# ZackAttack614/BlackBird

Hardware: AMD Instinct MI355X
Metric: selfplay_games_per_sec (higher is better)
Workload: dtype f32 (float32 operands split exactly into 3 bf16 values, 6 bf16 MFMA products each, f32 accumulate)

## Files before the change

### blackbird_amd/csrc/mega2.hip.h

```cpp
#pragma once
#include "net.hip.h"
#include "net_x3.hip.h"
#include "tree.hip.h"

#define MEGA_RMAX 4
#define MEGA_HEAD_FLOATS 192

#define MEGA2_QCAP 32
#ifndef BB_TREE_IDLE_SLEEP
#define BB_TREE_IDLE_SLEEP 4
#endif
#ifndef BB_NET_IDLE_SLEEP
#define BB_NET_IDLE_SLEEP 4
#endif

__device__ __forceinline__ int lds_load(volatile int *p) { return *p; }
__device__ __forceinline__ void release_global_then_lds() {
    __threadfence_block();
    asm volatile("s_waitcnt vmcnt(0)" ::: "memory");
}


template <class G, int GW, bool REC>
struct GameShadow {
    static constexpr int S = G::S, MP = G::MAXPATH;
    int32_t root[GW], root_N[GW], n_nodes[GW], ply[GW], sims_left[GW], pend_leaf[GW], pend_expand[GW], path_len[GW],
        game_lid[GW], sim_serial[GW], leaf_serial[GW], resume_cur[GW], resume_depth[GW], leaf_flags[GW];
    int32_t path_N[REC ? GW * MP : 1], path_all[REC ? GW * MP : 1];
    float path_W[REC ? GW * MP : 1];
    uint32_t leaf_game_id[GW];
    float root_W[GW], eval_value[GW];
    float eval_policy[GW * S];
    uint64_t evals[GW];
    uint64_t ctr[GW * 8];
    typename G::State leaf_state[GW];
    uint32_t path[GW * MP];
    int8_t root_pp[GW];

#define BB_SHADOW_ARRAYS(X)                                                                                           \
    X(root, 1) X(root_N, 1) X(n_nodes, 1) X(ply, 1) X(sims_left, 1) X(pend_leaf, 1) X(pend_expand, 1) X(path_len, 1)  \
    X(game_lid, 1) X(sim_serial, 1) X(leaf_serial, 1) X(resume_cur, 1) X(resume_depth, 1) X(leaf_game_id, 1)          \
    X(root_W, 1) X(eval_value, 1) X(eval_policy, S) X(evals, 1) X(ctr, 8) X(path, MP) X(root_pp, 1) X(leaf_flags, 1)
#define BB_SHADOW_REC_ARRAYS(X) X(path_N, MP) X(path_all, MP) X(path_W, MP)

    __device__ __forceinline__ void load(const TreeDev &d, int g0, int n, int nthreads) {
#define X(f, per) for (int i = threadIdx.x; i < n * (per); i += nthreads) f[i] = d.f[(size_t)g0 * (per) + i];
        BB_SHADOW_ARRAYS(X)
        if constexpr (REC) { BB_SHADOW_REC_ARRAYS(X) }
#undef X
        for (int i = threadIdx.x; i < n; i += nthreads) leaf_state[i] = ((const typename G::State *)d.leaf_state)[g0 + i];
    }
    __device__ __forceinline__ void store(const TreeDev &d, int g0, int n, int nthreads) {
#define X(f, per) for (int i = threadIdx.x; i < n * (per); i += nthreads) d.f[(size_t)g0 * (per) + i] = f[i];
        BB_SHADOW_ARRAYS(X)
        if constexpr (REC) { BB_SHADOW_REC_ARRAYS(X) }
#undef X
        for (int i = threadIdx.x; i < n; i += nthreads) ((typename G::State *)d.leaf_state)[g0 + i] = leaf_state[i];
    }
    __device__ __forceinline__ TreeDev local(const TreeDev &d, int g0) {
        TreeDev r = d;
#define X(f, per) r.f = f;
        BB_SHADOW_ARRAYS(X)
        if constexpr (REC) { BB_SHADOW_REC_ARRAYS(X) }
#undef X
        r.leaf_state = leaf_state;
        r.pool_g0 = g0;
        return r;
    }
};

struct QueueCtl {
    int q[MEGA2_QCAP];
    int head, tail, tree_done, abort_flag;
};

__device__ __attribute__((noinline)) int queue_pop(QueueCtl *c, long long t_start, long long t_limit, int n_tree) {
    int li = -1;
    if ((threadIdx.x & 63) == 0) {
        int h = lds_load(&c->head), t = lds_load(&c->tail);
        if (h < t) {
            if (atomicCAS(&c->head, h, h + 1) == h) {
                volatile int *slot = &c->q[h & (MEGA2_QCAP - 1)];
                for (int spin = 0; spin < (1 << 20) && (li = *slot) < 0; spin++) __builtin_amdgcn_s_sleep(1);
                *slot = -1;
                if (li < 0) {
                    c->abort_flag = 1;
                    li = -2;
                }
            }
        } else if (lds_load(&c->tree_done) >= n_tree) {
            li = -2;
        } else if (wall_clock64() - t_start > t_limit || lds_load(&c->abort_flag)) {
            c->abort_flag = 1;
            li = -2;
        }
    }
    return __builtin_amdgcn_readfirstlane(li);
}

template <bool GLOBAL_TOO>
__device__ __attribute__((noinline)) void queue_push(QueueCtl *c, uint8_t *state_byte, bool leader, bool posted, int li) {
    if (GLOBAL_TOO) release_global_then_lds();
    else __threadfence_block();
    if (leader) {
        if (posted) {
            *(volatile uint8_t *)state_byte = 1;
            int idx = atomicAdd(&c->tail, 1);
            *(volatile int *)&c->q[idx & (MEGA2_QCAP - 1)] = li;
        } else {
            *(volatile uint8_t *)state_byte = 0;
        }
    }
}

template <class G, int NETW, bool X3 = false, int WAVES = 12>
__global__ void __launch_bounds__(WAVES * 64) k_selfplay_queue(TreeDev dg, NetDev nd, NetX3 x3, int noise_on, int limit_s, int own_visits) {
    constexpr int MEGA2_THREADS = WAVES * 64;
    constexpr bool NET_APPLIES = !X3;
    constexpr int S = G::S, GW = 16, TREEW = WAVES - NETW, GPT = (GW + TREEW - 1) / TREEW;
    static_assert(GPT * S <= 64, "a tree wave holds at most 64 / S games");
    using NG = NetGeom<G, 1>;
    constexpr int RMAX = MEGA_RMAX, STEPS0 = NG::STEPS0;
    using XG = X3Geom<G>;
    constexpr int EPI_F = (1 + 2 * RMAX) * 48, HEAD_F = MEGA_HEAD_FLOATS;
    constexpr int WT_F = X3 ? 2 * RMAX * XG::LAYER12_B / 4 : 2 * RMAX * 9 * 64 * 4, W0_F = X3 ? XG::W0_B / 4 : STEPS0 * 64;
    constexpr int WAVE_F = X3 ? XG::WAVE_BYTES / 4 : NG::WAVE_FLOATS;
    __shared__ __attribute__((aligned(16))) float lds[NETW * WAVE_F];
    constexpr int WH_F = X3 ? 3 * 64 * 16 / 4 : 0;
    __shared__ __attribute__((aligned(16))) float wlds[WT_F + W0_F + EPI_F + HEAD_F + WH_F];
    __shared__ QueueCtl qc;
    __shared__ GameShadow<G, GW, X3> shadow;
    static_assert(GPT <= 8, "a tree wave's game states are one 8-byte word");
    __shared__ __attribute__((aligned(8))) uint8_t gstate[TREEW * 8];
#define GSI(li) ((((li) % TREEW) << 3) + (li) / TREEW)
    __shared__ int myslot[NETW];
    __shared__ int wg_pool, wg_dry, wg_refill;
    constexpr int CHUNK = GW * 32;
#ifdef BB_STAMPS
    __shared__ long long ts_post[GW], ts_done[GW];
#endif
    const int wave = threadIdx.x >> 6, l64 = threadIdx.x & 63;
    const int g0 = blockIdx.x * GW;
    const int n_mine = dg.n_slots - g0 < GW ? dg.n_slots - g0 : GW;
    shadow.load(dg, g0, n_mine, MEGA2_THREADS);
    const TreeDev d = shadow.local(dg, g0);
    if (threadIdx.x == 0) {
        qc.head = 0;
        qc.tail = 0;
        qc.tree_done = 0;
        qc.abort_flag = 0;
        wg_pool = n_mine * own_visits;
        wg_dry = 0;
        wg_refill = 0;
    }
    if (threadIdx.x < TREEW * 8) gstate[threadIdx.x] = 0;
#ifdef BB_STAMPS_NET
    if (threadIdx.x < 8) s_net_stamps[threadIdx.x] = 0;
#endif
    if (threadIdx.x < MEGA2_QCAP) qc.q[threadIdx.x] = -1;
    for (int i = threadIdx.x; i < NETW * WAVE_F; i += MEGA2_THREADS) lds[i] = 0.f;
    NetDev ndl = nd;
    NetX3 x3l = x3;
    {
        const float *gwt = X3 ? (const float *)x3.wt12 : (const float *)nd.wt;
        const float *gw0 = X3 ? (const float *)x3.w0 : nd.w0;
        const int wt_used = X3 ? 2 * nd.R * XG::LAYER12_B / 4 : 2 * nd.R * 9 * 64 * 4;
        for (int i = threadIdx.x; i < wt_used; i += MEGA2_THREADS) wlds[i] = gwt[i];
        for (int i = threadIdx.x; i < W0_F; i += MEGA2_THREADS) wlds[WT_F + i] = gw0[i];
        x3l.wt12 = (const unsigned char *)wlds;
        x3l.w0 = (const unsigned char *)(wlds + WT_F);
        for (int i = threadIdx.x; i < (1 + 2 * nd.R) * 48; i += MEGA2_THREADS) wlds[WT_F + W0_F + i] = nd.epi[i];
        for (int i = threadIdx.x; i < nd.head_floats; i += MEGA2_THREADS) wlds[WT_F + W0_F + EPI_F + i] = nd.head[i];
        if constexpr (X3) {
            for (int i = threadIdx.x; i < WH_F; i += MEGA2_THREADS) wlds[WT_F + W0_F + EPI_F + HEAD_F + i] = ((const float *)x3.wh)[i];
            x3l.wh = (const unsigned char *)(wlds + WT_F + W0_F + EPI_F + HEAD_F);
        }
        ndl.wt = (const f32x4 *)wlds;
        ndl.w0 = wlds + WT_F;
        ndl.epi = wlds + WT_F + W0_F;
        ndl.head = wlds + WT_F + W0_F + EPI_F;
    }
    __syncthreads();
    const long long t_start = wall_clock64();
    const long long t_limit = 100000000ll * limit_s;

    if (wave >= NETW) {
        const int tw = wave - NETW;
        __builtin_amdgcn_s_setprio(3);
        const int li = (l64 / S) * TREEW + tw, lane = l64 % S;
        const bool mine = l64 < GPT * S && li < GW && g0 + li < d.n_slots;
        const int g = li;
        bool alive = mine && d.game_lid[mine ? g : 0] >= 0;
#ifdef BB_STAMPS
        long long t_work = 0, t_all0 = clock64(), n_calls = 0, n_lanes = 0, t_pick = 0, n_pick = 0;
#endif
        auto early_post = [&](int gg, int ln) __attribute__((always_inline)) {
            if (NET_APPLIES) release_global_then_lds();
            else __threadfence_block();
            if (ln == 0) {
#ifdef BB_STAMPS
                ts_post[li] = wall_clock64();
#endif
                *(volatile uint8_t *)&gstate[GSI(li)] = 1;
                const int idx = atomicAdd(&qc.tail, 1);
                *(volatile int *)&qc.q[idx & (MEGA2_QCAP - 1)] = li;
            }
        };
        for (;;) {
            int stt = mine ? (int)*(volatile uint8_t *)&gstate[GSI(li)] : 1;
            const int pool = lds_load(&wg_pool), dry = lds_load(&wg_dry);
            if (pool < CHUNK / 4 && !dry && __any(alive)) {
                if (l64 == 0 && atomicCAS(&wg_refill, 0, 1) == 0) {
                    int old = atomicSub(d.visit_pool, CHUNK);
                    int got = old < 0 ? 0 : old < CHUNK ? old : CHUNK;
                    if (got) atomicAdd(&wg_pool, got);
                    else *(volatile int *)&wg_dry = 1;
                    __threadfence_block();
                    *(volatile int *)&wg_refill = 0;
                }
                if (pool <= 0) {
                    __builtin_amdgcn_s_sleep(1);
                    int late = wall_clock64() - t_start > t_limit || lds_load(&qc.abort_flag);
                    if (__builtin_amdgcn_readfirstlane(late)) {
                        qc.abort_flag = 1;
                        break;
                    }
                    continue;
                }
            }
            bool ready = mine && alive && pool > 0 && stt != 1;
            bool busy = mine && ((alive && pool > 0) || (alive && !dry) || stt == 1);
            if (!__any(busy)) break;
            if (__any(ready)) {
                __threadfence_block();
                bool posted = false;
#ifdef BB_STAMPS
                long long ts = clock64();
                n_calls++;
                n_lanes += __popcll(__ballot(ready)) / S;
                if (ready && lane == 0 && stt == 2) {
                    t_pick += wall_clock64() - ts_done[li];
                    n_pick++;
                }
#endif
#ifdef BB_STAMPS_LIGHT
                int ll = 0, lv = 0, lld = 0, lpu = 0;
                if (ready) {
                    posted = async_game<G, X3>(d, g, lane, ll, lv, lld, lpu, early_post);
                    if (d.game_lid[g] < 0) alive = false;
                }
                {
                    int m = lv;
                    for (int o = 32; o; o >>= 1) m = max(m, __shfl_xor(m, o, 64));
                    unsigned long long who = __ballot(ready && lane == 0 && lv == m);
                    if (who && l64 == (int)__builtin_ctzll(who) && d.stamps) {
                        atomicAdd(&d.stamps[6], (unsigned long long)ll);
                        atomicAdd(&d.stamps[7], (unsigned long long)lv);
                        atomicAdd(&d.stamps[11], (unsigned long long)lld);
                        atomicAdd(&d.stamps[12], (unsigned long long)lpu);
                    }
                }
#else
                if (ready) {
                    posted = async_game<G, X3>(d, g, lane, early_post);
                    if (d.game_lid[g] < 0) alive = false;
                }
#endif
                {
                    int used = __popcll(__ballot(ready && lane == 0));
                    if (l64 == 0) atomicSub(&wg_pool, used);
                }
                queue_push<NET_APPLIES>(&qc, &gstate[GSI(li < GW ? li : 0)], ready && lane == 0 && !posted, false, li);
#ifdef BB_STAMPS
                t_work += clock64() - ts;
#endif
            } else {
                __builtin_amdgcn_s_sleep(BB_TREE_IDLE_SLEEP);
                int late = wall_clock64() - t_start > t_limit || lds_load(&qc.abort_flag);
                if (__builtin_amdgcn_readfirstlane(late)) {
                    qc.abort_flag = 1;
                    break;
                }
            }
        }
        if (l64 == 0) atomicAdd(&qc.tree_done, 1);
#ifdef BB_STAMPS
        if (l64 == 0 && d.stamps) {
            atomicAdd(&d.stamps[2], (unsigned long long)t_work);
            atomicAdd(&d.stamps[3], (unsigned long long)(clock64() - t_all0));
            atomicAdd(&d.stamps[5], 1ull);
            atomicAdd(&d.stamps[13], (unsigned long long)n_calls);
            atomicAdd(&d.stamps[14], (unsigned long long)n_lanes);
        }
        if (lane == 0 && d.stamps && n_pick) {
            atomicAdd(&d.stamps[8], (unsigned long long)t_pick);
            atomicAdd(&d.stamps[9], (unsigned long long)n_pick);
        }
#endif
    } else {
        float *wl = lds + wave * WAVE_F;
        constexpr bool CACHE = X3 && G::CACHE_KEY;
        const EvalCache ecache = {(u32x4 *)dg.eval_cache, dg.eval_cache_log2};
        unsigned long long n_probes = 0, n_hits = 0;
#ifdef BB_STAMPS
        long long t_work = 0, t_all0 = clock64(), n_evals = 0, t_qwait = 0;
#endif
        for (;;) {
            const int li = __builtin_amdgcn_readfirstlane(queue_pop(&qc, t_start, t_limit, TREEW));
            if (li == -2) break;
            if (li < 0) {
                __builtin_amdgcn_s_sleep(BB_NET_IDLE_SLEEP);
                continue;
            }
            __threadfence_block();
#ifdef BB_STAMPS
            long long ts = clock64();
            n_evals++;
            t_qwait += wall_clock64() - ts_post[li];
#endif
            if (l64 == 0) myslot[wave] = li;
            if constexpr (X3) {
                int probe = -1;
                net_body_x3<G, true, false, CACHE>(ndl, x3l, 1, 0, &myslot[wave], (unsigned char *)wl, (const typename G::State *)d.leaf_state, nullptr,
                                     d.leaf_game_id, d.leaf_serial, noise_on, d.eval_value, nullptr, d.eval_policy, S, false, nullptr,
                                     ecache, &probe);
                if constexpr (CACHE) {
                    n_probes += probe >= 0;
                    if (probe > 0) {
                        n_hits++;
                        if (l64 == 0) d.evals[li] -= 1;
                    }
                }
            } else
                net_body<G, 1, 2>(ndl, 1, 0, &myslot[wave], wl, (const typename G::State *)d.leaf_state, nullptr,
                                  d.leaf_game_id, d.leaf_serial, noise_on, d.eval_value, nullptr, d.eval_policy, S, false);
            if constexpr (NET_APPLIES) {
            __threadfence_block();
#ifdef BB_STAMPS_NET
            long long _na = clock64();
#endif
            if (l64 < S) {
                phase_apply<G>(d, li, l64);
                if (l64 == 0) d.sims_left[li] -= 1;
            }
#ifdef BB_STAMPS_NET
            if (l64 == 0) atomicAdd(&s_net_stamps[5], (unsigned long long)(clock64() - _na));
#endif
            }
            release_global_then_lds();
#ifdef BB_STAMPS
            if (l64 == 0) ts_done[li] = wall_clock64();
#endif
            if (l64 == 0) *(volatile uint8_t *)&gstate[GSI(li)] = 2;
#ifdef BB_STAMPS
            t_work += clock64() - ts;
#endif
        }
#ifdef BB_STAMPS
        if (l64 == 0 && d.stamps) {
            atomicAdd(&d.stamps[0], (unsigned long long)t_work);
            atomicAdd(&d.stamps[1], (unsigned long long)(clock64() - t_all0));
            atomicAdd(&d.stamps[4], 1ull);
            atomicAdd(&d.stamps[15], (unsigned long long)n_evals);
            atomicAdd(&d.stamps[10], (unsigned long long)t_qwait);
        }
#endif
        if (CACHE && l64 == 0 && n_probes && dg.eval_cache_ctr) {
            atomicAdd(&dg.eval_cache_ctr[0], n_hits);
            atomicAdd(&dg.eval_cache_ctr[1], n_probes);
        }
    }
    __syncthreads();
#ifdef BB_STAMPS_NET
    if (threadIdx.x < 8) atomicAdd(&g_net_stamps[threadIdx.x], s_net_stamps[threadIdx.x]);
#endif
    if (qc.abort_flag) {
        if (threadIdx.x == 0) d.ctr[6] += 1;
        if ((int)threadIdx.x < n_mine && gstate[GSI(threadIdx.x)] == 1) shadow.pend_leaf[threadIdx.x] = -1;
    }
    __syncthreads();
    shadow.store(dg, g0, n_mine, MEGA2_THREADS);
}
```

### blackbird_amd/csrc/tree.hip.h

```cpp
#pragma once
#include "games.hip.h"
#include "rng.hip.h"

#define NODE_EXPANDED 1
#define NODE_TERMINAL 2
#define NODE_CACHED 4
#define LEAF_RECORDED 0x40000000
#define CHILD_NONE (-1)
#define CHILD_TERM_BIT 0x40000000

template <class G>
struct alignas(128) DenseNode {
    int32_t flags;
    uint32_t legal_mask;
    int32_t all;
    int32_t serial;
    double sq;
    double pad0;
    int32_t N[G::S];
    float Q[G::S];
    int32_t child[G::S];
    alignas(128) double cP[G::S];
    float W[G::S];
    typename G::State st;
// ... 696 lines not shown
    pool->serial = 0;
    d.n_nodes[g] = 1;
    d.root[g] = 0;
    d.root_N[g] = 0;
    d.root_W[g] = 0.f;
    d.root_pp[g] = 0;
    d.ply[g] = 0;
    d.pend_leaf[g] = -1;
    d.pend_expand[g] = 0;
    d.path_len[g] = 0;
    d.sim_serial[g] = 0;
    d.game_lid[g] = lid;
    if (d.leaf_flags) d.leaf_flags[g] = 0;
    if (d.track_anc) {
        d.anc_len[g] = 0;
        d.top_N[g] = 0;
    }
}

template <class G>
__global__ void __launch_bounds__(256) k_set_roots(TreeDev d, int n, const int32_t *slots,
                                                   const typename G::State *states, const uint32_t *game_ids) {
    int i = blockIdx.x * blockDim.x + threadIdx.x;
    if (i >= n) return;
    int g = slots ? slots[i] : i;
    if (g < 0 || g >= d.n_slots) return;
    reset_slot<G>(d, g, game_ids ? (int)game_ids[i] : g, states[i]);
    d.sims_left[g] = 0;
}

template <class G>
__global__ void __launch_bounds__(256) k_add_sims(TreeDev d, int sims, const uint8_t *mask = nullptr) {
    int g = blockIdx.x * blockDim.x + threadIdx.x;
    if (g >= d.n_slots) return;
    if (d.game_lid[g] >= 0 && (!mask || mask[g])) d.sims_left[g] = sims;
}

template <class G>
__global__ void __launch_bounds__(256) k_get_roots(TreeDev d, typename G::State *out) {
    int g = blockIdx.x * blockDim.x + threadIdx.x;
    if (g >= d.n_slots) return;
    out[g] = ((DenseNode<G> *)d.nodes + (size_t)(g + d.pool_g0) * d.node_cap + d.root[g])->st;
}

template <class G>
__global__ void __launch_bounds__(256) k_selfplay_begin(TreeDev d) {
    int g = blockIdx.x * blockDim.x + threadIdx.x;
    if (g >= d.n_slots) return;
    if (g + d.slot_offset < d.n_games_target) {
        reset_slot<G>(d, g, g + d.slot_offset, G::initial());
        d.sims_left[g] = d.sims_per_move;
    } else {
        reset_slot<G>(d, g, -1, G::initial());
        d.sims_left[g] = 0;
    }
}

template <class G>
__device__ __forceinline__ uint8_t *example_ptr(const TreeDev &d, int lid, int ply) {
    return d.examples + ((size_t)lid * (d.max_plies + 1) + ply) * d.example_bytes;
}

template <class G>
__device__ __forceinline__ void write_example(const TreeDev &d, int lid, int ply, const typename G::State &st, int lane, int Ni,
                              int total, uint32_t gid) {
    uint8_t *p = example_ptr<G>(d, lid, ply);
    if (lane == 0) {
        ExampleHdr h;
        h.game_id = gid;
        h.ply = (uint16_t)ply;
        h.player = (uint8_t)gs_player(st);
        h.z = 0;
        h.total = (uint32_t)total;
        h.n_children = G::A;
        *(ExampleHdr *)p = h;
        *(typename G::State *)(p + sizeof(ExampleHdr)) = st;
    }
    ((uint32_t *)(p + sizeof(ExampleHdr) + sizeof(typename G::State)))[lane] = (uint32_t)Ni;
}

template <class G>
__device__ __forceinline__ void selfplay_move_body(const TreeDev &d, int g, int lane) {
    using Node = DenseNode<G>;
    constexpr int S = G::S;
    int lid = d.game_lid[g];
    if (lid < 0) return;
    Node *pool = (Node *)d.nodes + (size_t)(g + d.pool_g0) * d.node_cap;
    typename G::State st = pool[d.root[g]].st;
    uint32_t gid = d.first_game_id + (uint32_t)lid;
    int ply = d.ply[g];
    double u = bb_u53(d.seed, gid, (uint32_t)ply);
    int total, Ni;
    float Wi;
    int act = choose_move<G>(d, g, lane, d.temp, u, total, Ni, Wi);
    if (act < 0) {
        if (lane == 0) {
            d.game_lid[g] = -1;
            d.ctr[(size_t)g * 8 + 6] += 1;
        }
        return;
    }
    write_example<G>(d, lid, ply, st, lane, Ni, total, gid);
    typename G::State ns;
    advance_root<G>(d, g, lane, act, ns);
    __threadfence_block();
    ply += 1;
    int w = G::winner(ns, -1);
    bool over = w >= 0 || ply >= d.max_plies;
    if (!over) {
        if (lane == 0) {
            d.ply[g] = ply;
            d.sims_left[g] = d.sims_per_move;
            d.ctr[(size_t)g * 8 + 5] += 1;
        }
        return;
    }
    write_example<G>(d, lid, ply, ns, lane, 0, 0, gid);
    __threadfence_block();
    for (int k = lane; k <= ply; k += S) {
        ExampleHdr *h = (ExampleHdr *)example_ptr<G>(d, lid, k);
        h->z = (w <= 0) ? 0 : (h->player == w ? 1 : -1);
    }
    __threadfence();
    if (lane == 0) {
        int32_t *gh = d.game_hdr + (size_t)lid * 4;
        gh[0] = ply + 1;
        gh[1] = w;
        gh[2] = ply;
        __threadfence();
        gh[3] = 1;
        uint64_t *c = d.ctr + (size_t)g * 8;
        c[4] += 1;
        c[5] += 1;
        c[7] += (uint64_t)(ply + 1);
        int next = lid + d.lid_stride;
        if (next < d.n_games_target) {
            reset_slot<G>(d, g, next, G::initial());
            d.sims_left[g] = d.sims_per_move;
        } else {
            d.game_lid[g] = -1;
            d.sims_left[g] = 0;
        }
    }
}

template <class G>
__global__ void __launch_bounds__(256) k_selfplay_move(TreeDev d) {
    constexpr int S = G::S;
    int t = blockIdx.x * blockDim.x + threadIdx.x;
    int g = t / S, lane = t % S;
    if (g >= d.n_slots) return;
    phase_apply<G>(d, g, lane);
    __threadfence_block();
    selfplay_move_body<G>(d, g, lane);
}

struct NoPostHook {
    __device__ __forceinline__ void operator()(int, int) const {}
};
template <class G, bool REC = false, class OnPost = NoPostHook>
__device__ bool async_game(const TreeDev &d, int g, int lane
#ifdef BB_STAMPS_LIGHT
                           , int &g_light_loop, int &g_light_levels, int &g_light_load, int &g_light_puct
#endif
                           , OnPost on_post = OnPost()) {
    using Node = DenseNode<G>;
    constexpr int S = G::S, A = G::A;
    if (d.game_lid[g] < 0) return false;
    Node *pool = (Node *)d.nodes + (size_t)(g + d.pool_g0) * d.node_cap;
#ifdef BB_STAMPS_LIGHT
    int lt_in = (int)clock64(), lt_loop = 0, ln_levels = 0, lt_create = 0, lt_puct = 0;
#endif
    if (d.pend_leaf[g] >= 0) {
        if (REC && (d.leaf_flags[g] & LEAF_RECORDED)) phase_apply_rec<G>(d, g, lane);
        else phase_apply<G>(d, g, lane);
        if (lane == 0) d.sims_left[g] -= 1;
        __threadfence_block();
    }
    int budget = d.level_budget;
    uint32_t *path = d.path + (size_t)g * G::MAXPATH;
    int sims_done = 0, depth_sum = 0, term_hits = 0;
    bool posted = false;
    for (;;) {
        if (d.sims_left[g] <= 0) {
            selfplay_move_body<G>(d, g, lane);
            __threadfence_block();
            if (d.game_lid[g] < 0) break;
        }
        int cur = d.resume_cur[g], depth = 0;
        if (cur >= 0) depth = d.resume_depth[g];
        else cur = d.root[g];
        int nn = d.n_nodes[g];
        typename G::State st;
        int flags = 0;
        enum { F_PARKED = 2, F_LEAF = 4, F_TERM = 8, F_EXPAND = 16, F_OVERFLOW = 32 };
        int fl = 0;
#ifdef BB_STAMPS_LIGHT
        int lt_e = (int)clock64();
#endif
        for (;;) {
            if (budget <= 0) { fl |= F_PARKED; break; }
            budget--;
#ifdef BB_STAMPS_LIGHT
            ln_levels++;
            int lt_a = (int)clock64();
#endif
            Node *node = pool + cur;
            typename G::State st_l = node->st;
            int flags_l = node->flags;
            uint32_t mask = node->legal_mask;
            double sq = node->sq;
            int Ni = node->N[lane];
            float Qi = node->Q[lane];
            double cPi = node->cP[lane];
            int ci = node->child[lane];
            double cached = node->pad0;
            float Wi = 0.f;
            int all_l = 0;
            if (REC) {
                Wi = node->W[lane];
                all_l = node->all;
            }
            asm volatile("" ::"v"(flags_l), "v"(mask), "v"(sq), "v"(Ni), "v"(Qi), "v"(cPi), "v"(ci));
#ifdef BB_STAMPS_LIGHT
            int lt_b = (int)clock64();
            lt_create += lt_b - lt_a;
#endif
            st = st_l;
            flags = flags_l;
            if (!(flags & NODE_EXPANDED)) {
                fl |= F_LEAF;
                if (flags & NODE_TERMINAL) {
                    fl |= F_TERM;
                    if (flags & NODE_CACHED) {
                        float v01 = (float)cached;
                        __threadfence_block();
                        if (REC) backup_path_rec<G>(d, g, lane, pool, depth, v01, gs_prev(st));
                        else backup_path<G>(d, g, lane, pool, depth, v01, gs_prev(st));
                        if (lane == 0) d.sims_left[g] -= 1;
                        __threadfence_block();
                        sims_done++;
                        depth_sum += depth;
                        term_hits++;
                        fl &= ~F_LEAF;
                    }
                } else {
                    fl |= F_EXPAND;
                }
                break;
            }
            static_assert(G::MAXPATH >= G::H * G::W + 2, "a descent places at most H*W stones");
            int child = ci;
            int a = grp_argmax_puct<S>(Qi, cPi, sq, Ni, lane < A && ((mask >> lane) & 1u), child);
#ifdef BB_STAMPS_LIGHT
            asm volatile("" ::"v"(a), "v"(child));
            lt_puct += (int)clock64() - lt_b;
#endif
            if (lane == 0) path[depth] = ((uint32_t)cur << 6) | ((uint32_t)((flags >> 4) & 3) << 4) | (uint32_t)a;
            if (REC) {
                if (lane == 0) d.path_all[(size_t)g * G::MAXPATH + depth] = all_l;
                if (lane == a) {
                    d.path_N[(size_t)g * G::MAXPATH + depth] = Ni;
                    d.path_W[(size_t)g * G::MAXPATH + depth] = Wi;
                }
            }
            if (child == CHILD_NONE) {
                typename G::State st2;
                bool terminal;
                child = create_child<G>(d, g, pool, node, st, a, lane, nn, st2, terminal, &flags);
                if (child == CHILD_NONE) { fl |= F_OVERFLOW | F_LEAF; break; }
                st = st2;
                depth++;
                cur = child & ~CHILD_TERM_BIT;
                fl |= F_LEAF | (terminal ? F_TERM : F_EXPAND);
                break;
            }
            depth++;
            cur = child & ~CHILD_TERM_BIT;
        }
#ifdef BB_STAMPS_LIGHT
        lt_loop += (int)clock64() - lt_e;
#endif
        if (lane == 0) {
            d.resume_cur[g] = (fl & F_PARKED) ? cur : -1;
            d.resume_depth[g] = (fl & F_PARKED) ? depth : 0;
        }
        if (fl & F_PARKED) break;
        if (!(fl & F_LEAF)) {
            if (lane == 0) d.sim_serial[g] += 1;
            continue;
        }
        if (lane == 0) {
            ((typename G::State *)d.leaf_state)[g] = st;
            d.leaf_game_id[g] = d.first_game_id + (uint32_t)d.game_lid[g];
            d.leaf_serial[g] = cur;
            d.pend_leaf[g] = cur;
            if (d.leaf_flags) d.leaf_flags[g] = REC ? (flags | LEAF_RECORDED) : 0;
            d.pend_expand[g] = (fl & F_EXPAND) ? 1 : 0;
            d.path_len[g] = depth;
            d.sim_serial[g] += 1;
            d.evals[g] += 1;
            d.ctr[(size_t)g * 8 + 6] += (uint64_t)((fl & F_OVERFLOW) ? 1 : 0);
        }
        on_post(g, lane);
        sims_done++;
        depth_sum += depth;
        term_hits += (fl & F_TERM) ? 1 : 0;
        posted = true;
        break;
    }
#ifdef BB_STAMPS_LIGHT
    g_light_loop = lt_loop;
    g_light_load = lt_create;
    g_light_puct = lt_puct;
    g_light_levels = ln_levels;
    (void)lt_in;
#endif
    if (lane == 0 && sims_done) {
        uint64_t *c = d.ctr + (size_t)g * 8;
        c[0] += (uint64_t)sims_done;
        c[1] += (uint64_t)depth_sum;
        c[3] += (uint64_t)term_hits;
    }
    return posted;
}

template <class G>
__global__ void __launch_bounds__(256) k_tree_async(TreeDev d, int round) {
    constexpr int S = G::S;
    int t = blockIdx.x * blockDim.x + threadIdx.x;
    int wv = t >> 6, l64 = t & 63;
    int g = wv * d.gpw + l64 / S, lane = l64 % S;
    bool live = l64 < d.gpw * S && g < d.n_slots;
#ifdef BB_STAMPS_LIGHT
    int ll = 0, lv = 0, lld = 0, lpu = 0;
    bool posted = live ? async_game<G>(d, g, lane, ll, lv, lld, lpu) : false;
    {
        int m = lv;
        for (int o = 32; o; o >>= 1) m = max(m, __shfl_xor(m, o, 64));
        unsigned long long who = __ballot(live && lane == 0 && lv == m);
        if (who && l64 == (int)__builtin_ctzll(who) && d.stamps) {
            atomicAdd(&d.stamps[6], (unsigned long long)ll);
            atomicAdd(&d.stamps[7], (unsigned long long)lv);
            atomicAdd(&d.stamps[11], (unsigned long long)lld);
            atomicAdd(&d.stamps[12], (unsigned long long)lpu);
        }
    }
#else
    bool posted = live ? async_game<G>(d, g, lane) : false;
#endif
    unsigned long long m = __ballot(posted && lane == 0);
    if (t == 0) d.post_count[(round + 2) & 3] = 0;
    if (m) {
        int leader = __ffsll((long long)m) - 1;
        int base = 0;
        if (l64 == leader) base = atomicAdd(&d.post_count[round & 3], __popcll(m));
        base = __shfl(base, leader, 64);
        if (posted && lane == 0) d.post_slot[base + __popcll(m & ((1ull << l64) - 1ull))] = g;
    }
}
```

Before: 9406.

## Let tree waves dynamically claim any ready game instead of fixed home games

Result: faster. 9849, median of 6 (+4.7%).

```diff
diff --git a/blackbird_amd/csrc/mega2.hip.h b/blackbird_amd/csrc/mega2.hip.h
--- a/blackbird_amd/csrc/mega2.hip.h
+++ b/blackbird_amd/csrc/mega2.hip.h
@@ -98,19 +98,73 @@
     return __builtin_amdgcn_readfirstlane(li);
 }
 
-template <bool GLOBAL_TOO>
-__device__ __attribute__((noinline)) void queue_push(QueueCtl *c, uint8_t *state_byte, bool leader, bool posted, int li) {
-    if (GLOBAL_TOO) release_global_then_lds();
-    else __threadfence_block();
-    if (leader) {
-        if (posted) {
-            *(volatile uint8_t *)state_byte = 1;
-            int idx = atomicAdd(&c->tail, 1);
-            *(volatile int *)&c->q[idx & (MEGA2_QCAP - 1)] = li;
-        } else {
-            *(volatile uint8_t *)state_byte = 0;
-        }
-    }
+struct TreeCtl {
+    int state[16];
+    int pool, dry, refill;
+};
+#define MEGA2_CLAIM 6
+#define MEGA2_CLAIM_STOP 0x100u
+
+__device__ __attribute__((noinline)) void tree_unclaim(int *state, bool leader) {
+    release_global_then_lds();
+    if (leader) *(volatile int *)state = 0;
+}
+
+template <int CLAIM, int TREEW, int GW, int CHUNK>
+__device__ __attribute__((noinline)) unsigned long long tree_claim(TreeCtl *c_, QueueCtl *q_, const int32_t *game_lid_, int *visit_pool,
+                                                                   int n_mine, int tw, long long t_start, long long t_limit) {
+    static_assert(GW == 16 && CLAIM <= 8, "sixteen state words, eight nibbles");
+    TreeCtl *c = as_lds(c_);
+    QueueCtl *q = as_lds(q_);
+    const int32_t *game_lid = as_lds(game_lid_);
+    const int l = threadIdx.x & 63;
+    const bool in = l < n_mine;
+    const int pool = lds_load(&c->pool), dry = lds_load(&c->dry);
+    const int st = in ? lds_load(&c->state[l]) : 0;
+    const bool alive = in && game_lid[in ? l : 0] >= 0;
+    int idle = BB_TREE_IDLE_SLEEP;
+    if (pool < CHUNK / 4 && !dry && __any(alive)) {
+        if (l == 0 && atomicCAS(&c->refill, 0, 1) == 0) {
+            int old = atomicSub(visit_pool, CHUNK);
+            int got = old < 0 ? 0 : old < CHUNK ? old : CHUNK;
+            if (got) atomicAdd(&c->pool, got);
+            else *(volatile int *)&c->dry = 1;
+            __threadfence_block();
+            *(volatile int *)&c->refill = 0;
+        }
+        if (pool <= 0) idle = 1;
+    }
+    const bool ready = alive && pool > 0 && (st == 0 || st == 2);
+    const bool busy = in && ((alive && (pool > 0 || !dry)) || st == 1 || st == 3);
+    if (!__any(busy)) return (unsigned long long)MEGA2_CLAIM_STOP << 32;
+    const unsigned ready_m = (unsigned)__ballot(ready);
+    if (ready_m) {
+        unsigned home0 = 0;
+        for (int k = 0; k * TREEW < GW; k++) home0 |= 1u << (k * TREEW);
+        const unsigned home = (home0 << tw) & ((1u << GW) - 1u);
+        const int quota = CLAIM - __popc(ready_m & home);
+        const unsigned others = ready_m & ~home;
+        const int r = (tw + 1) & (GW - 1);
+        const unsigned rot = ((others >> r) | (others << (GW - r))) & ((1u << GW) - 1u);
+        const int rank = __popc(rot & ((1u << ((l - r) & (GW - 1))) - 1u));
+        const bool take = ready && (((home >> (l & (GW - 1))) & 1u) || rank < quota);
+        bool won = false;
+        if (take) won = atomicCAS(&c->state[l], st, 3) == st;
+        unsigned won_m = (unsigned)__ballot(won);
+        if (won_m) {
+            unsigned packed = 0, n = 0;
+            for (; won_m; won_m &= won_m - 1u, n++) packed |= (unsigned)__builtin_ctz(won_m) << (4 * n);
+            return ((unsigned long long)n << 32) | packed;
+        }
+    }
+    if (idle == 1) __builtin_amdgcn_s_sleep(1);
+    else __builtin_amdgcn_s_sleep(BB_TREE_IDLE_SLEEP);
+    const int late = wall_clock64() - t_start > t_limit || lds_load(&q->abort_flag);
+    if (__builtin_amdgcn_readfirstlane(late)) {
+        q->abort_flag = 1;
+        return (unsigned long long)MEGA2_CLAIM_STOP << 32;
+    }
+    return 0;
 }
 
 template <class G, int NETW, bool X3 = false, int WAVES = 12>
@@ -130,11 +184,10 @@
     __shared__ __attribute__((aligned(16))) float wlds[WT_F + W0_F + EPI_F + HEAD_F + WH_F];
     __shared__ QueueCtl qc;
     __shared__ GameShadow<G, GW, X3> shadow;
-    static_assert(GPT <= 8, "a tree wave's game states are one 8-byte word");
-    __shared__ __attribute__((aligned(8))) uint8_t gstate[TREEW * 8];
-#define GSI(li) ((((li) % TREEW) << 3) + (li) / TREEW)
+    constexpr int CLAIM = 64 / S < MEGA2_CLAIM ? 64 / S : MEGA2_CLAIM;
+    static_assert(CLAIM >= GPT, "a tree wave can always hold its home games");
+    __shared__ TreeCtl tc;
     __shared__ int myslot[NETW];
-    __shared__ int wg_pool, wg_dry, wg_refill;
     constexpr int CHUNK = GW * 32;
 #ifdef BB_STAMPS
     __shared__ long long ts_post[GW], ts_done[GW];
@@ -149,11 +202,14 @@
         qc.tail = 0;
         qc.tree_done = 0;
         qc.abort_flag = 0;
-        wg_pool = n_mine * own_visits;
-        wg_dry = 0;
-        wg_refill = 0;
-    }
-    if (threadIdx.x < TREEW * 8) gstate[threadIdx.x] = 0;
+        tc.pool = n_mine * own_visits;
+        tc.dry = 0;
+        tc.refill = 0;
+    }
+    if (threadIdx.x < GW) tc.state[threadIdx.x] = 0;
+#ifdef BB_STAMPS
+    if (threadIdx.x < GW) ts_done[threadIdx.x] = 0;
+#endif
 #ifdef BB_STAMPS_NET
     if (threadIdx.x < 8) s_net_stamps[threadIdx.x] = 0;
 #endif
@@ -187,101 +243,65 @@
     if (wave >= NETW) {
         const int tw = wave - NETW;
         __builtin_amdgcn_s_setprio(3);
-        const int li = (l64 / S) * TREEW + tw, lane = l64 % S;
-        const bool mine = l64 < GPT * S && li < GW && g0 + li < d.n_slots;
-        const int g = li;
-        bool alive = mine && d.game_lid[mine ? g : 0] >= 0;
+        const int grp = l64 / S, lane = l64 % S;
 #ifdef BB_STAMPS
         long long t_work = 0, t_all0 = clock64(), n_calls = 0, n_lanes = 0, t_pick = 0, n_pick = 0;
 #endif
         auto early_post = [&](int gg, int ln) __attribute__((always_inline)) {
-            if (NET_APPLIES) release_global_then_lds();
-            else __threadfence_block();
+            release_global_then_lds();
             if (ln == 0) {
 #ifdef BB_STAMPS
-                ts_post[li] = wall_clock64();
-#endif
-                *(volatile uint8_t *)&gstate[GSI(li)] = 1;
+                ts_post[gg] = wall_clock64();
+#endif
+                *(volatile int *)&tc.state[gg] = 1;
                 const int idx = atomicAdd(&qc.tail, 1);
-                *(volatile int *)&qc.q[idx & (MEGA2_QCAP - 1)] = li;
+                *(volatile int *)&qc.q[idx & (MEGA2_QCAP - 1)] = gg;
             }
         };
         for (;;) {
-            int stt = mine ? (int)*(volatile uint8_t *)&gstate[GSI(li)] : 1;
-            const int pool = lds_load(&wg_pool), dry = lds_load(&wg_dry);
-            if (pool < CHUNK / 4 && !dry && __any(alive)) {
-                if (l64 == 0 && atomicCAS(&wg_refill, 0, 1) == 0) {
-                    int old = atomicSub(d.visit_pool, CHUNK);
-                    int got = old < 0 ? 0 : old < CHUNK ? old : CHUNK;
-                    if (got) atomicAdd(&wg_pool, got);
-                    else *(volatile int *)&wg_dry = 1;
-                    __threadfence_block();
-                    *(volatile int *)&wg_refill = 0;
+#ifdef BB_STAMPS
+            const long long ts = clock64();
+#endif
+            const unsigned long long cl = tree_claim<CLAIM, TREEW, GW, CHUNK>(&tc, &qc, d.game_lid, d.visit_pool, n_mine, tw, t_start, t_limit);
+            const unsigned games = __builtin_amdgcn_readfirstlane((unsigned)cl), hi = __builtin_amdgcn_readfirstlane((unsigned)(cl >> 32));
+            if (hi & MEGA2_CLAIM_STOP) break;
+            const int n = (int)(hi & 15u);
+            if (!n) continue;
+            const bool ready = grp < n;
+            const int g = (int)((games >> (4 * (grp & 7))) & 15u);
+            __threadfence_block();
+            bool posted = false;
+#ifdef BB_STAMPS
+            n_calls++;
+            n_lanes += n;
+            if (ready && lane == 0 && ts_done[g]) {
+                t_pick += wall_clock64() - ts_done[g];
+                n_pick++;
+                ts_done[g] = 0;
+            }
+#endif
+#ifdef BB_STAMPS_LIGHT
+            int ll = 0, lv = 0, lld = 0, lpu = 0;
+            if (ready) posted = async_game<G, X3>(d, g, lane, ll, lv, lld, lpu, early_post);
+            {
+                int m = lv;
+                for (int o = 32; o; o >>= 1) m = max(m, __shfl_xor(m, o, 64));
+                unsigned long long who = __ballot(ready && lane == 0 && lv == m);
+                if (who && l64 == (int)__builtin_ctzll(who) && d.stamps) {
+                    atomicAdd(&d.stamps[6], (unsigned long long)ll);
+                    atomicAdd(&d.stamps[7], (unsigned long long)lv);
+                    atomicAdd(&d.stamps[11], (unsigned long long)lld);
+                    atomicAdd(&d.stamps[12], (unsigned long long)lpu);
                 }
-                if (pool <= 0) {
-                    __builtin_amdgcn_s_sleep(1);
-                    int late = wall_clock64() - t_start > t_limit || lds_load(&qc.abort_flag);
-                    if (__builtin_amdgcn_readfirstlane(late)) {
-                        qc.abort_flag = 1;
-                        break;
-                    }
-                    continue;
-                }
-            }
-            bool ready = mine && alive && pool > 0 && stt != 1;
-            bool busy = mine && ((alive && pool > 0) || (alive && !dry) || stt == 1);
-            if (!__any(busy)) break;
-            if (__any(ready)) {
-                __threadfence_block();
-                bool posted = false;
-#ifdef BB_STAMPS
-                long long ts = clock64();
-                n_calls++;
-                n_lanes += __popcll(__ballot(ready)) / S;
-                if (ready && lane == 0 && stt == 2) {
-                    t_pick += wall_clock64() - ts_done[li];
-                    n_pick++;
-                }
-#endif
-#ifdef BB_STAMPS_LIGHT
-                int ll = 0, lv = 0, lld = 0, lpu = 0;
-                if (ready) {
-                    posted = async_game<G, X3>(d, g, lane, ll, lv, lld, lpu, early_post);
-                    if (d.game_lid[g] < 0) alive = false;
-                }
-                {
-                    int m = lv;
-                    for (int o = 32; o; o >>= 1) m = max(m, __shfl_xor(m, o, 64));
-                    unsigned long long who = __ballot(ready && lane == 0 && lv == m);
-                    if (who && l64 == (int)__builtin_ctzll(who) && d.stamps) {
-                        atomicAdd(&d.stamps[6], (unsigned long long)ll);
-                        atomicAdd(&d.stamps[7], (unsigned long long)lv);
-                        atomicAdd(&d.stamps[11], (unsigned long long)lld);
-                        atomicAdd(&d.stamps[12], (unsigned long long)lpu);
-                    }
-                }
+            }
 #else
-                if (ready) {
-                    posted = async_game<G, X3>(d, g, lane, early_post);
-                    if (d.game_lid[g] < 0) alive = false;
-                }
-#endif
-                {
-                    int used = __popcll(__ballot(ready && lane == 0));
-                    if (l64 == 0) atomicSub(&wg_pool, used);
-                }
-                queue_push<NET_APPLIES>(&qc, &gstate[GSI(li < GW ? li : 0)], ready && lane == 0 && !posted, false, li);
-#ifdef BB_STAMPS
-                t_work += clock64() - ts;
-#endif
-            } else {
-                __builtin_amdgcn_s_sleep(BB_TREE_IDLE_SLEEP);
-                int late = wall_clock64() - t_start > t_limit || lds_load(&qc.abort_flag);
-                if (__builtin_amdgcn_readfirstlane(late)) {
-                    qc.abort_flag = 1;
-                    break;
-                }
-            }
+            if (ready) posted = async_game<G, X3>(d, g, lane, early_post);
+#endif
+            if (l64 == 0) atomicSub(&tc.pool, n);
+            tree_unclaim(&tc.state[g], ready && lane == 0 && !posted);
+#ifdef BB_STAMPS
+            t_work += clock64() - ts;
+#endif
         }
         if (l64 == 0) atomicAdd(&qc.tree_done, 1);
 #ifdef BB_STAMPS
@@ -351,7 +371,7 @@
 #ifdef BB_STAMPS
             if (l64 == 0) ts_done[li] = wall_clock64();
 #endif
-            if (l64 == 0) *(volatile uint8_t *)&gstate[GSI(li)] = 2;
+            if (l64 == 0) *(volatile int *)&tc.state[li] = 2;
 #ifdef BB_STAMPS
             t_work += clock64() - ts;
 #endif
@@ -376,7 +396,7 @@
 #endif
     if (qc.abort_flag) {
         if (threadIdx.x == 0) d.ctr[6] += 1;
-        if ((int)threadIdx.x < n_mine && gstate[GSI(threadIdx.x)] == 1) shadow.pend_leaf[threadIdx.x] = -1;
+        if ((int)threadIdx.x < n_mine && tc.state[threadIdx.x] == 1) shadow.pend_leaf[threadIdx.x] = -1;
     }
     __syncthreads();
     shadow.store(dg, g0, n_mine, MEGA2_THREADS);
diff --git a/blackbird_amd/csrc/tree.hip.h b/blackbird_amd/csrc/tree.hip.h
--- a/blackbird_amd/csrc/tree.hip.h
+++ b/blackbird_amd/csrc/tree.hip.h
@@ -1022,10 +1022,17 @@
             d.evals[g] += 1;
             d.ctr[(size_t)g * 8 + 6] += (uint64_t)((fl & F_OVERFLOW) ? 1 : 0);
         }
-        on_post(g, lane);
         sims_done++;
         depth_sum += depth;
         term_hits += (fl & F_TERM) ? 1 : 0;
+        if (lane == 0) {
+            uint64_t *c = d.ctr + (size_t)g * 8;
+            c[0] += (uint64_t)sims_done;
+            c[1] += (uint64_t)depth_sum;
+            c[3] += (uint64_t)term_hits;
+        }
+        sims_done = 0;
+        on_post(g, lane);
         posted = true;
         break;
     }
```
